# personalrobotics/or_cdchomp

Hardware: AMD Instinct MI355X
Metric: CHOMP iters/sec, 7-DOF x 100-waypoint (higher is better)
Workload: dtype f64; 1 GPU; WAM 7-DOF, n_points=100, batch=1024 random adofgoal per GPU, n_iter=100 per step, lambda=100 obs_factor=500, tabletop SDF 40x31x12 (BASELINE configs[1]); runs_per_gpu=1024, n_iter=100, n_points=100, dof=7, parallelism=runs sharded over 1 GPU(s) in contiguous blocks, no collective

## Files before the change

### or_cdchomp_amd/csrc/batch.cpp

```cpp
#include "module.h"
#include "kernel_table.h"
#include "launch.h"
#include "verdict_device.h"
#include <algorithm>
#include <cmath>
#include <cstring>
#include <functional>
#include <stdexcept>
#include <thread>
#include <exception>
#include <cstdlib>

hipError_t orc_launch_hmc_seed(uint32_t * state, int * next, const unsigned int * seeds, int n_runs, hipStream_t stream);
hipError_t orc_launch_hmc_plan_f64(uint32_t * state, int * next, int n_runs, int iter_begin, int iter_end, int cap, size_t mn, double lambda,
   double * noise, int * iters, int * overflow, hipStream_t stream);
hipError_t orc_launch_hmc_plan_f32(uint32_t * state, int * next, int n_runs, int iter_begin, int iter_end, int cap, size_t mn, double lambda,
   float * noise, int * iters, int * overflow, hipStream_t stream);
size_t orc_perturb_lds_bytes(int m, int n);
hipError_t orc_launch_perturb_f64(double * traj, int n_runs, int n_points, int n, int m, const unsigned int * seeds, int D,
   const double * genU, const double * genV, double scale, const double * lim_lo, const double * lim_hi, size_t lds, hipStream_t stream);
hipError_t orc_launch_perturb_f32(float * traj, int n_runs, int n_points, int n, int m, const unsigned int * seeds, int D,
   const double * genU, const double * genV, double scale, const double * lim_lo, const double * lim_hi, size_t lds, hipStream_t stream);
hipError_t orc_launch_select_best(const double * costs, const int * status, const unsigned long long * verdict_key, const int * group, int n_runs, int column,
   unsigned long long * key, int * count, int * best, hipStream_t stream);
// ... 479 lines not shown
   std::vector<int> flat((size_t) n_runs * maxr, -1);
   for (int k=0; k<n_runs; k++) for (size_t r=0; r<iters[k].size(); r++) flat[(size_t) k*maxr + r] = iters[k][r];
   if (flat.size() > hmc_cap_iters_)
   {
      own_hmc_iters_.reset(); own_hmc_iters_.reset(dev_alloc<int>(flat.size())); d_hmc_iters_ = own_hmc_iters_.as<int>(); hmc_cap_iters_ = flat.size();
   }
   hip_check(hipMemcpyAsync(d_hmc_iters_, flat.data(), flat.size()*sizeof(int), hipMemcpyHostToDevice, stream_), "hmc iters");
   const size_t ncount = (size_t) n_runs * maxr * mn;
   const size_t rsize = (params.precision == 64) ? 8 : 4;
   if (ncount * rsize > noise_cap_)
   {
      own_noise_.reset(); own_noise_.reset(dev_alloc<char>(ncount * rsize)); d_noise_ = own_noise_.as<void>(); noise_cap_ = ncount * rsize;
   }
   if (params.precision == 64)
   {
      std::vector<double> buf(ncount, 0.0);
      parallel_for_runs(n_runs, [&](int k_lo, int k_hi) {
         for (int k=k_lo; k<k_hi; k++) std::copy(noise[k].begin(), noise[k].end(), buf.begin() + (size_t) k*maxr*mn);
      });
      hip_check(hipMemcpyAsync(d_noise_, buf.data(), ncount*8, hipMemcpyHostToDevice, stream_), "noise");
      hip_check(hipStreamSynchronize(stream_), "noise sync");
   }
   else
   {
      std::vector<float> buf(ncount, 0.f);
      for (int k=0; k<n_runs; k++)
         for (size_t e=0; e<noise[k].size(); e++) buf[(size_t) k*maxr*mn + e] = (float) noise[k][e];
      hip_check(hipMemcpyAsync(d_noise_, buf.data(), ncount*4, hipMemcpyHostToDevice, stream_), "noise");
      hip_check(hipStreamSynchronize(stream_), "noise sync");
   }
}

template <typename real>
void BatchShard::launch(int n_iter, bool final_eval, bool carry)
{
   const IteratePlan & P = plan_;
   DevBatch<real> b;
   std::memset(&b, 0, sizeof(b));
   b.model = d_model_.as<const DevModel<real>>();
   b.sdfs = d_sdfs_.as<const DevSdf<real>>();
   b.sdfc = d_sdfc_.as<const DevSdfCell<real>>();
   b.n_sdfs = scn_.n_sdfs;
   b.scene_of_run = d_scene_of_run_.as<int>(); b.scene_nsdf = d_scene_nsdf_.as<int>(); b.n_scenes = scn_.n_scenes; b.sdfc_stride = scn_.sdfc_stride;
   b.n_runs = n_runs; b.n_points = m + 2; b.np_global = n_points; b.free_start = params.free_start; b.m = m; b.n = n;
   if (params.free_start && P.tile_first < 2)
      throw std::runtime_error("start_tsr: the first tile must hold the two points after the start point!");
   b.tile_m = P.tile_m;
   b.n_tiles = P.n_tiles; b.tile_first = P.tile_first; b.tile_rest = P.tile_rest;
   if (!P.g_in_lds && !d_Gcost_) d_Gcost_.reset(dev_alloc<real>((size_t) n_runs * m * n));
   b.traj = d_traj_.as<real>(); b.AG = d_AG_.as<real>(); b.Gcost = d_Gcost_.as<real>();
   b.Gdbg = sw_.debug_state ? d_G_.as<real>() : nullptr;
   b.g_in_lds = P.g_in_lds; b.lds_flags = P.lds_flags; b.t_in_lds = P.t_in_lds; b.t_staged = (P.lds_flags & ORC_LDS_T_STAGED) ? 1 : 0;
   b.ms = ms_;
   b.lay = P.lay;
   b.costs = d_costs_.as<double>(); b.trace = d_trace_.as<double>(); b.status = d_status_.as<int>(); b.iters_done = d_iters_done_.as<int>();
   b.leapfrog_first = d_leap_.as<int>();
   const double dt = 1.0/(n_points-1);
   b.dt = (real) dt;
   b.inv_2dt = (real)(1.0/(2.0*dt));
   b.inv_dt2 = (real)(1.0/(dt*dt));
   b.shared.lambda = (real) params.lambda;
   b.inv_m = (real)(1.0/m);
   b.shared.epsilon = (real) params.epsilon; b.epsilon_self = (real) params.epsilon_self;
   b.shared.obs_factor = (real) params.obs_factor; b.shared.obs_factor_self = (real) params.obs_factor_self;
   b.run_params = run_params_on_ ? d_run_params_.as<const RunParams<real>>() : nullptr;
   b.use_momentum = params.use_momentum; b.use_hmc = params.use_hmc && max_resamples_ > 0;
   b.D = (params.derivative == 1 && params.free_start) ? -1 : params.derivative;
   b.Aband = d_Aband_.as<const real>(); b.beta_s = d_beta_s_.as<const real>(); b.beta_g = d_beta_g_.as<const real>();
   b.metric64 = d_metric64_.as<const double>();
   b.kss = metric_.kss; b.ksg = metric_.ksg; b.kgg = metric_.kgg;
   b.solve_mode = met_.solve_mode;
   b.pcr_levels = metric_.pcr_levels;
   b.pcr = d_pcr_.as<const real>(); b.Ainv = d_Ainv_.as<const real>();
   b.ss_rank = (met_.solve_mode == 3) ? metric_.ss_rank : 0;
   b.jl_lo = d_jl_lo_.as<const real>(); b.jl_hi = d_jl_hi_.as<const real>();
   b.hmc_iters = d_hmc_iters_; b.noise = (const real *) d_noise_; b.max_resamples = max_resamples_;
   b.n_iter = n_iter; b.final_eval = final_eval ? 1 : 0; b.carry_status = carry ? 1 : 0;
   b.conv_patience = conv.patience > 0 ? conv.patience : 0;
   b.conv_rtol = conv.rtol; b.conv_obs_max = conv.obs_max;
   b.conv_prev = d_conv_prev_.as<double>(); b.conv_streak = d_conv_streak_.as<int>();
   b.phase_cycles = d_phase_.as<long long>();
   b.pcr_in_lds = P.pcr_in_lds; b.pcr_sym = met_.pcr_sym; b.pcr_rows = met_.pcr_rows; b.ag_in_lds = P.ag_in_lds;
   b.stagger_mode = sw_.stagger_mode; b.stagger_sleeps = sw_.stagger_sleeps; b.lim_generic = sw_.lim_generic;
   b.band_toeplitz = met_.band_toeplitz;
   for (int k=0; k<=ORC_SS_MAX_RANK; k++) { b.band_c64[k] = met_.band_c64[k]; b.band_c[k] = (real) met_.band_c64[k]; }
   if (params.derivative == 1 && m >= 2)
   {
      b.a_diag = (real) metric_.Adense[(size_t) 1*m + 1];
      b.a_off = (real) metric_.Adense[(size_t) 1*m + 0];
   }
   else if (params.derivative == 1)
   {
      b.a_diag = (real) metric_.Adense[0];
      b.a_off = (real) metric_.beta_s[0];
   }
   b.tsrs = d_tsrs_.as<const DevTsr<real>>(); b.n_tsrs = tsr_.n_tsrs; b.cons_k = tsr_.cons_k; b.tsr_blocks = tsr_.blocks;
   b.tsr_structured = P.tsr_structured; b.tsr_wcap = P.tsr_wcap; b.tsr_nmax = P.tsr_nmax;
   b.tsr_ws = d_tsr_ws_.as<real>(); b.tsr_ws_stride = tsr_.ws_stride; b.tsr_err = d_tsr_err_.as<int>();
   hipEvent_t ev[2] = { mod_->acquire_event(device), mod_->acquire_event(device) };
   hip_check(hipEventRecord(ev[0], stream_), "hipEventRecord");
   hipError_t e = orc_launch_iterate(b, P.lds_bytes, stream_, P.variant, P.block);
   hip_check(e, "chomp_iterate_kernel launch");
   hip_check(hipEventRecord(ev[1], stream_), "hipEventRecord");
   pending_events_.push_back(std::make_pair(ev[0], ev[1]));
}

void BatchShard::iterate_async(int n_iter, int iter_begin, bool final_eval, bool carry)
{
   if (n_iter < 0) throw std::runtime_error("n_iter must be >=0!");
   if (unusable_) throw std::runtime_error("hmc: an earlier iterate call of this batch ran out of room for its momentum resamples; destroy the batch and create it again!");
   DeviceGuard guard(device);
   last_n_iter = n_iter;
   const size_t tneed = (size_t) n_runs * (n_iter ? n_iter : 1) * 3;
   if (tneed > trace_cap_)
   {
      hip_check(hipStreamSynchronize(stream_), "sync");
      d_trace_.reset(); d_trace_.reset(dev_alloc<double>(tneed)); trace_cap_ = tneed;
   }
   max_resamples_ = 0;
   if (iter_begin == 0) std::fill(ext_noise_used_.begin(), ext_noise_used_.end(), 0);
   std::unique_lock<std::mutex> plan_lock;
   if (params.use_hmc && n_iter > 0 && hmc_on_device_) plan_lock = std::unique_lock<std::mutex>(mod_->plan_buffers(device, stream_).enqueue);
   if (params.use_hmc && n_iter > 0) plan_hmc(iter_begin, iter_begin + n_iter);
   if (params.precision == 64) launch<double>(n_iter, final_eval, carry); else launch<float>(n_iter, final_eval, carry);
}

void BatchShard::sync_begin(double * costs_out, int * status_out, int * iters_out)
{
   DeviceGuard guard(device);
   hipStream_t st = stream_;
   if (costs_out) hip_check(hipMemcpyAsync(costs_out, d_costs_.as<void>(), (size_t) n_runs*3*sizeof(double), hipMemcpyDeviceToHost, st), "costs");
   if (status_out) hip_check(hipMemcpyAsync(status_out, d_status_.as<void>(), n_runs*sizeof(int), hipMemcpyDeviceToHost, st), "status");
   if (iters_out) hip_check(hipMemcpyAsync(iters_out, d_iters_done_.as<void>(), n_runs*sizeof(int), hipMemcpyDeviceToHost, st), "iters_done");
   if (overflow_armed_)
   {
      hip_check(hipMemcpyAsync(&overflow_host_, d_overflow_.as<void>(), sizeof(int), hipMemcpyDeviceToHost, st), "hmc overflow");
      hip_check(hipMemsetAsync(d_overflow_.as<void>(), 0, sizeof(int), st), "hmc overflow");
   }
}

void BatchShard::sync_end()
{
   DeviceGuard guard(device);
   hip_check(hipStreamSynchronize(stream_), "hipStreamSynchronize");
   harvest_events(false);
   if (overflow_armed_ && overflow_host_)
   {
      overflow_host_ = 0;
      unusable_ = true;
      throw std::runtime_error("hmc: a run drew more momentum resamples in one iterate call than the plan has room for (probability ~1e-12 per run and call); "
                               "the batch is not usable any more: destroy it, create it again and iterate with fewer iterations per call!");
   }
}

namespace {
void download(void * d, size_t count, int precision, double * out, hipStream_t st)
{
   if (precision == 64)
   {
      hip_check(hipMemcpyAsync(out, d, count*sizeof(double), hipMemcpyDeviceToHost, st), "download");
      hip_check(hipStreamSynchronize(st), "sync");
   }
   else
   {
      std::vector<float> tmp(count);
      hip_check(hipMemcpyAsync(tmp.data(), d, count*sizeof(float), hipMemcpyDeviceToHost, st), "download");
// ... 519 lines not shown
```

### or_cdchomp_amd/csrc/chomp_kernel.hip

```cpp
#include <hip/hip_runtime.h>
#include <math.h>
#include <atomic>
#include <type_traits>
#include <utility>
#include "dev_types.h"
#include "kernel_table.h"
#include "launch.h"

#pragma clang fp contract(fast)


namespace {

#include "sdf_lookup.h"

__device__ __forceinline__ double rcp_fast(double x)
{
   double r = __builtin_amdgcn_rcp(x);
   r = fma(fma(-x, r, 1.0), r, r);
   r = fma(fma(-x, r, 1.0), r, r);
   return r;
}
__device__ __forceinline__ float rcp_fast(float x) { return 1.0f / x; }
__device__ __forceinline__ double sqrt_rsq(double x, double * inv)
// ... 1468 lines not shown
         __syncthreads();
      }
   }
   if (staged)
   {
      copy_batched<real, BLOCK>(E.traj_g + n, T_s + n, mn);
      __syncthreads();
   }
   phase_mark<real>(b, E, 4);
   if (b.phase_cycles && tid == 0) E.phc_s[6] += num_limadjs;
   return num_limadjs;
}

struct PassCosts { double obs, smooth; };
template <typename real, bool GS16, int BLOCK, int WGS = 0>
__device__ __attribute__((noinline)) PassCosts phase_costs(const void * kp, int do_iteration_in, double cost_lane)
{
   KArg<real> & b = *uniform_kernarg<real>(kp);
   const bool do_iteration = uni(do_iteration_in) != 0;
   const Env<real> E = make_env<real, GS16>(b, orc_smem);
   const int tid = threadIdx.x;
   const int n = b.n, m = b.m, np = b.n_points, mn = m*n;
   const float rn_f = 1.0f / (float) n;
   const real * T_s = E.T_u;
   const bool staged = !b.t_in_lds && b.t_staged;
   if (staged && !do_iteration)
   {
      copy_batched<real, BLOCK>(E.T_u, E.traj_g, np*n);
      __syncthreads();
   }
   PassCosts pc;
   __builtin_amdgcn_s_setprio(PRIO_UPDATE);
   {
      double acc = 0.0;
      if (b.D != 1) acc = band_cost_pass<real, BLOCK>(kp, E.pcr_tab, T_s);
      else
      for (int e=tid; e<mn; e+=BLOCK)
      {
         const int i = div_n(e, rn_f), c = e - i*n;
         const real sg = smooth_grad<real>(b, T_s, i, c);
         const real bt = b.a_off * ((i == 0 ? T_s[c] : (real)0) + (i == m-1 ? T_s[(np-1)*n + c] : (real)0));
         acc += (double) T_s[n + e] * (0.5 * ((double) sg + (double) bt));
      }
      double ss = 0.0, sg2 = 0.0, gg = 0.0;
      if (tid < n)
      {
         const double s0 = (double) T_s[tid], g0 = (double) T_s[(np-1)*n + tid];
         ss = s0*s0; sg2 = s0*g0; gg = g0*g0;
      }
      acc += 0.5 * (b.kss*ss + 2.0*b.ksg*sg2 + b.kgg*gg);
      const double a = wave_sum(cost_lane), c2 = wave_sum(acc);
      __syncthreads();
      if ((tid & 63) == 0) { E.red[tid >> 6] = a; E.red[8 + (tid >> 6)] = c2; }
      __syncthreads();
      pc.obs = sum_partials<BLOCK>(E.red);
      pc.smooth = sum_partials<BLOCK>(E.red + 8);
      pc.obs /= (double) m;
   }
   phase_mark<real>(b, E, 5);

   if (do_iteration && b.free_start)
   {
      real * Tw = E.T_s;
      if (tid < n) Tw[tid] = Tw[2*n + tid];
      __syncthreads();
   }
   if (do_iteration && E.mod.floating)
   {
      real * Tw = E.T_u;
      for (int w=tid; w<np; w+=BLOCK)
      {
         real * row = Tw + w*n;
         const real len = M<real>::sqrt_(row[3]*row[3] + row[4]*row[4] + row[5]*row[5] + row[6]*row[6]);
         const real inv = (real)1 / len;
         row[3] *= inv; row[4] *= inv; row[5] *= inv; row[6] *= inv;
         if (staged) { real * g = E.traj_g + w*n; g[3] = row[3]; g[4] = row[4]; g[5] = row[5]; g[6] = row[6]; }
      }
      __syncthreads();
   }
   if (b.conv_patience && do_iteration) conv_step<real>(b, pc.obs, pc.smooth);
   return pc;
}

template <typename real, bool GS16, int BLOCK, int WGS = 0>
__device__ __attribute__((noinline)) void phase_finish(const void * kp, int status_in, int iters_done_in, int leapfrog_first_in, int have_costs_in,
   double done_obs, double done_smooth)
{
   KArg<real> & b = *uniform_kernarg<real>(kp);
   int status = uni(status_in);
   const int iters_done = uni(iters_done_in), leapfrog_first = uni(leapfrog_first_in), have_costs = uni(have_costs_in);
   const Env<real> E = make_env<real, GS16>(b, orc_smem);
   const int run = blockIdx.x, tid = threadIdx.x;
   const int n = b.n, m = b.m, np = b.n_points, mn = m*n;
   __syncthreads();
   if (b.conv_patience)
   {
      const ConvState * cs = conv_state();
      if (status == 0 && uni(cs->streak) >= b.conv_patience) status = 1;
      if (tid == 0) { b.conv_prev[run] = cs->prev; b.conv_streak[run] = cs->streak; }
   }
   if (b.t_in_lds)
   {
      const int skip = b.free_start ? n : 0;
      for (int e=skip+tid; e<np*n; e+=BLOCK) E.traj_g[e - skip] = E.T_s[e];
   }
   if (b.use_momentum && b.ag_in_lds) for (int e=tid; e<mn; e+=BLOCK) E.AG_g[e] = E.AG_s[e];
   if (tid == 0)
   {
      if (b.phase_cycles) for (int k=0; k<8; k++) b.phase_cycles[(size_t) run*8 + k] = E.phc_s[k];
      if (have_costs)
      {
         b.costs[(size_t) run*3 + 0] = done_obs + done_smooth;
         b.costs[(size_t) run*3 + 1] = done_obs;
         b.costs[(size_t) run*3 + 2] = done_smooth;
      }
      b.status[run] = status;
      b.iters_done[run] = (b.carry_status ? b.iters_done[run] : 0) + iters_done;
      b.leapfrog_first[run] = leapfrog_first;
   }
   if (b.trace && status != 0)
      for (int e=iters_done*3 + tid; e<b.n_iter*3; e+=BLOCK)
         b.trace[(size_t) run * b.n_iter * 3 + e] = __longlong_as_double(0x7ff8000000000000LL);
}

template <typename real, bool TREE, bool GS16, int BLOCK, int KIND = 0, int WGS = 0>
__global__ __launch_bounds__(BLOCK, (WGS ? WGS : orc::waves_per_simd(sizeof(real), GS16, BLOCK)))
void chomp_iterate_kernel(const DevBatch<real> b)
{
   const void * kp = (const void *) __builtin_amdgcn_kernarg_segment_ptr();
   const int run = blockIdx.x;
   const int tid = threadIdx.x;

   if (b.carry_status && b.status[run] != 0 && (b.status[run] != 1 || b.n_iter != 0)) return;

   phase_setup<real, TREE, GS16, BLOCK, WGS>(kp);

   int leapfrog_first = uni(b.leapfrog_first[run]);
   int status = 0;
   int next_resample = 0;

   if (b.stagger_mode && b.stagger_mode != 9)
   {
      const bool late = (b.stagger_mode == 1) ? (blockIdx.x & 1) : ((blockIdx.x >> 8) & 1);
      if (late) for (int k=0; k<b.stagger_sleeps; k++) __builtin_amdgcn_s_sleep(127);
   }

   double done_obs = 0.0, done_smooth = 0.0;
   int have_costs = 0;
   int iters_done = 0;
   const int total_passes = b.n_iter + (b.final_eval ? 1 : 0);

   for (int it=0; it<total_passes; it++)
   {
      const bool do_iteration = (it < b.n_iter);
      if (do_iteration && uni(conv_state()->stop)) continue;

      if (do_iteration && b.use_hmc && b.use_momentum && next_resample < b.max_resamples
          && b.hmc_iters[(size_t) run * b.max_resamples + next_resample] == it)
      {
         phase_hmc<real, GS16, BLOCK, WGS>(kp, next_resample);
         leapfrog_first = 1;
         next_resample++;
      }

      double cost_lane = 0.0;
      for (int tk=0; tk<b.n_tiles; tk++)
      {
         const int ts = (tk == 0) ? 0 : b.tile_first + (tk - 1) * b.tile_rest;
         const int te = (tk == b.n_tiles - 1) ? b.m : b.tile_first + tk * b.tile_rest;
         if (b.stagger_mode == 9 && tk > 0) { if (tk == 1) for (int k=0; k<b.stagger_sleeps; k++) __builtin_amdgcn_s_sleep(10); continue; }
#ifndef ORC_ABLATE_FK
         if (!b.ms.fk_split && uni(tid >> 6) * 20 >= te - ts + 2) __syncthreads();
         else phase_fk<real, TREE, GS16, BLOCK, WGS>(kp, ts, te);
#ifdef ORC_ABLATE_FKTWICE
         phase_fk<real, TREE, GS16, BLOCK, WGS>(kp, ts, te);
#endif
#endif
#ifndef ORC_ABLATE_COST
         if (do_iteration && !GS16) cost_lane = phase_cost_body<real, TREE, GS16, BLOCK, KIND, true>(kp, ts, te, cost_lane);
         else
         cost_lane = do_iteration ? phase_cost<real, TREE, GS16, BLOCK, KIND, true, WGS>(kp, ts, te, cost_lane)
                                  : phase_cost<real, TREE, GS16, BLOCK, KIND, false, WGS>(kp, ts, te, cost_lane);
         if (tk == 0 && b.free_start) cost_lane = phase_cost_start<real, TREE, GS16, BLOCK, WGS>(kp, do_iteration ? 1 : 0, cost_lane);
#endif
      }

      if (do_iteration)
      {
         const bool lean = b.solve_mode == 2 && b.n <= 64 && !b.lim_generic && b.Gdbg == nullptr;
         const int num_limadjs = !lean ? uni(phase_update<real, TREE, GS16, BLOCK, WGS, 0>(kp, it, leapfrog_first))
                               : (b.n_tsrs == 0 ? uni(phase_update<real, TREE, GS16, BLOCK, WGS, 1>(kp, it, leapfrog_first))
                                                : uni(phase_update<real, TREE, GS16, BLOCK, WGS, 2>(kp, it, leapfrog_first)));
         if (b.use_momentum) leapfrog_first = 0;
         if (!(num_limadjs < 1000)) status = -1;
      }
      if (status != 0) break;

      PassCosts pc = phase_costs<real, GS16, BLOCK, WGS>(kp, do_iteration ? 1 : 0, cost_lane);
      pc.obs = unir(pc.obs); pc.smooth = unir(pc.smooth);

      if (tid == 0 && b.trace && do_iteration)
      {
         double * tr = b.trace + ((size_t) run * b.n_iter + it) * 3;
         tr[0] = pc.obs + pc.smooth; tr[1] = pc.obs; tr[2] = pc.smooth;
      }
      done_obs = pc.obs; done_smooth = pc.smooth; have_costs = 1;
      if (do_iteration) iters_done++;

   }

   phase_finish<real, GS16, BLOCK, WGS>(kp, status, iters_done, leapfrog_first, have_costs, done_obs, done_smooth);
}

template <typename real>
__global__ void seed_traj_kernel(real * traj, const double * starts, const double * goals,
   int n_runs, int n_points, int n, int floating)
{
   const long total = (long) n_runs * n_points;
   for (long idx = blockIdx.x * (long) blockDim.x + threadIdx.x; idx < total; idx += (long) gridDim.x * blockDim.x)
   {
      const int run = (int)(idx / n_points);
      const int i = (int)(idx - (long) run * n_points);
      double row[ORC_MAX_JOINTS + 7];
      for (int j=0; j<n; j++)
      {
         const double s = starts[(size_t) run*n + j];
         const double g = goals[(size_t) run*n + j];
         row[j] = s + (g - s) * i / (n_points - 1);
      }
      if (floating)
      {
         const double len = ::sqrt(__dadd_rn(__dadd_rn(__dadd_rn(__dmul_rn(row[3], row[3]), __dmul_rn(row[4], row[4])), __dmul_rn(row[5], row[5])), __dmul_rn(row[6], row[6])));
         const double inv = 1.0 / len;
         row[3] *= inv; row[4] *= inv; row[5] *= inv; row[6] *= inv;
      }
      for (int j=0; j<n; j++) traj[((size_t) run * n_points + i) * n + j] = (real) row[j];
   }
}

template <typename real, bool TREE>
__global__ __launch_bounds__(ORC_BLOCK)
void collision_verdict_kernel(DevVerdict<real> v)
{
   extern __shared__ __align__(16) unsigned char smem_raw[];
   const DevModel<real> & gmod = *v.model;
   const int run = blockIdx.x, tid = threadIdx.x;
   const int n = v.n, np = v.n_points, nj = gmod.nj, Sa = gmod.Sa;
   const int pstr = (Sa*3) | 1, astr = (nj*6) | 1, chunk = v.chunk;
   const int scene = v.scene_of_run ? v.scene_of_run[run] : 0;
   const int n_fields = v.scene_nsdf ? v.scene_nsdf[scene] : v.n_sdfs;
   const DevSdf<real> * sdfs = v.sdfs + (size_t) scene * v.n_sdfs;
   unsigned long long * key_s = (unsigned long long *) smem_raw;
   real * lds = (real *)(smem_raw + 16);
   real * rows_s = lds;
   real * pos_s = rows_s + ((chunk*n + 3) & ~3);
   real * ax_s = pos_s + ((chunk*pstr + 3) & ~3);
   real * base_s = ax_s + ((chunk*astr + 3) & ~3);
   real * srad_s = base_s + 12;
   int * slot_s = (int *)(srad_s + ((Sa + 3) & ~3));
   int * xml_s = slot_s + ((gmod.Sa_real + 3) & ~3);
   int * jctl_s = xml_s + ((Sa + 3) & ~3);
   for (int e=tid; e<12; e+=ORC_BLOCK) base_s[e] = (e < 9) ? gmod.base_R[e] : gmod.base_t[e-9];
   for (int e=tid; e<Sa; e+=ORC_BLOCK) { srad_s[e] = gmod.sph_radius[e]; xml_s[e] = v.slot_xml[e]; }
   for (int e=tid; e<gmod.Sa_real; e+=ORC_BLOCK) slot_s[e] = gmod.slot_of[e];
   for (int e=tid; e<nj; e+=ORC_BLOCK) { jctl_s[2*e] = gmod.joints[e].packed; jctl_s[2*e+1] = 0; }
   if (tid == 0) key_s[0] = ORC_VERDICT_NONE;
   ModelView<real> mod;
   mod.nj = nj; mod.n = n; mod.floating = gmod.floating; mod.tree = gmod.tree; mod.Sa = Sa; mod.S = gmod.S; mod.GS = gmod.GS;
   mod.base_sph_begin = gmod.base_sph_begin; mod.base_sph_end = gmod.base_sph_end; mod.jt_scan = 0;
   mod.Sa_real = gmod.Sa_real; mod.placed = gmod.placed; mod.live_mask = gmod.live_mask; mod.slot_of = slot_s;
   mod.base_R = base_s; mod.base_t = base_s + 9;
   mod.jctl = jctl_s; mod.sph_affects = nullptr; mod.n_static = 0; mod.empty_mask = 0u;
   mod.jpk = (const __attribute__((address_space(4))) int *) gmod.jpacked;
   mod.jpk2 = (const __attribute__((address_space(4))) int *) gmod.jpacked2;
   mod.sph_pos_c = (const __attribute__((address_space(4))) real (*)[3]) gmod.sph_pos;
   mod.joints_c = (const __attribute__((address_space(4))) DevJoint<real> *) gmod.joints;
   mod.slot_c = (const __attribute__((address_space(4))) int *) gmod.slot_of;
   mod.fkj = (const __attribute__((address_space(4))) DevFkJoint<real> *) gmod.fkj;
   __syncthreads();

   const real * traj = v.traj + (size_t) run * np * n;
   const int s0 = v.offs[run], s1 = v.offs[run+1];
   double my_depth = 0.0; unsigned long long my_key = ORC_VERDICT_NONE;
   for (int base=s0; base<s1; base+=chunk)
   {
      const int count = (s1 - base < chunk) ? s1 - base : chunk;
      for (int e=tid; e<count*n; e+=ORC_BLOCK)
      {
         const int s = e / n, c = e - s*n;
         const int sg = v.seg[base + s];
         const real uu = v.u[base + s];
// ... 145 lines not shown
```

### or_cdchomp_amd/csrc/dev_types.h

```cpp
#pragma once
#include <cstddef>

#define ORC_MAX_JOINTS   32
#define ORC_MAX_SPHERES  64
#define ORC_MAX_POINTS   4096
#define ORC_MAX_SAVE     4
#define ORC_MAX_SDFS     8
#define ORC_BLOCK        256
#ifndef ORC_WGS_PER_CU
#define ORC_WGS_PER_CU    3
#endif
#ifndef ORC_WGS_PER_CU_FP32_MANY
#define ORC_WGS_PER_CU_FP32_MANY 4
#endif
#define ORC_SS_MAX_RANK   4
#define ORC_SCAN_RPL      4
#define ORC_VERDICT_NONE  0x7fffffffffffffffull
#define ORC_LDS_HEADER    256
#define ORC_LIM_LIST      64
#define ORC_LIM_SCRATCH  (256 + ORC_LIM_LIST*16)
#define ORC_PAIR_ROUNDS   16
#define ORC_PAIR_DEG      4

enum : int
// ... 150 lines not shown
struct RunParams
{
   real lambda, epsilon, obs_factor, obs_factor_self;
};

template <typename real>
struct DevBatch
{
   ModelScalars ms;
   LdsLayout lay;
   const DevModel<real> * model;
   const DevSdf<real> * sdfs;
   const DevSdfCell<real> * sdfc;
   int n_sdfs;
   const int * scene_of_run;
   const int * scene_nsdf;
   int n_scenes, sdfc_stride;
   int n_runs, n_points, m, n;
   int tile_m;
   int n_tiles;
   int tile_first, tile_rest;
   real * traj;
   real * AG;
   real * Gdbg;
   real * Gcost;
   double * costs;
   double * trace;
   int * status;
   int * iters_done;
   int * leapfrog_first;
   real dt, inv_2dt, inv_dt2, inv_m;
   real epsilon_self;
   RunParams<real> shared;
   const RunParams<real> * run_params;
   int use_momentum, use_hmc, D;
   const real * Aband;
   const real * beta_s;
   const real * beta_g;
   const double * metric64;
   double kss, ksg, kgg;
   int solve_mode;
   int pcr_levels;
   const real * pcr;
   const real * Ainv;
   const real * jl_lo;
   const real * jl_hi;
   const int * hmc_iters;
   const real * noise;
   int max_resamples;
   int n_iter;
   int final_eval;
   int carry_status;
   long long * phase_cycles;
   real a_diag, a_off;
   int pcr_in_lds;
   int t_in_lds;
   int t_staged;
   int g_in_lds;
   int lds_flags;
   int ag_in_lds;
   int pcr_sym;
   int pcr_rows;
   int lim_generic;
   int stagger_mode;
   int stagger_sleeps;
   const DevTsr<real> * tsrs;
   int n_tsrs, cons_k;
   int tsr_blocks;
   int tsr_structured;
   int tsr_wcap;
   int tsr_nmax;
   int free_start, np_global;
   real * tsr_ws;
   size_t tsr_ws_stride;
   int * tsr_err;
   int band_toeplitz;
   real band_c[ORC_SS_MAX_RANK + 1];
   double band_c64[ORC_SS_MAX_RANK + 1];
   int ss_rank;
   int conv_patience;
   double conv_rtol, conv_obs_max;
   double * conv_prev;
   int * conv_streak;
};

template <typename real>
struct DevVerdict
{
   const DevModel<real> * model;
   const DevSdf<real> * sdfs;
   int n_sdfs;
   const int * scene_of_run;
   const int * scene_nsdf;
   int n_runs, n_points, n;
   int chunk;
   const real * traj;
   const int * offs;
   const int * seg;
   const real * u;
   const int * slot_xml;
   int n_pairs;
   const int * pairs;
   const real * pair_rsum;
   const real * inact_pos;
   unsigned long long * key_out;
   double * depth_out;
};


template <typename real>
struct ModelView
{
   int nj, n, floating, tree, Sa, S, GS, base_sph_begin, base_sph_end, jt_scan, Sa_real, placed, n_static;
   unsigned int empty_mask;
   unsigned long long live_mask;
   const int * slot_of;
   const real * base_R;
   const real * base_t;
   const int * jctl;
   const unsigned long long * sph_affects;
   const unsigned long long * sph_allowed;
   const __attribute__((address_space(4))) int * jpk;
   const __attribute__((address_space(4))) int * jpk2;
   const __attribute__((address_space(4))) real (* sph_pos_c)[3];
   const __attribute__((address_space(4))) int * slot_c;
   const __attribute__((address_space(4))) DevJoint<real> * joints_c;
   const __attribute__((address_space(4))) DevFkJoint<real> * fkj;
   const __attribute__((address_space(4))) int * static_slot_c;
   const __attribute__((address_space(4))) real (* static_pos_c)[3];
   const __attribute__((address_space(4))) RunParams<real> * rp;
   int n_sdfs;
   const __attribute__((address_space(4))) DevSdfCell<real> * sdfc;
};
#if defined(__HIPCC__)
__host__ __device__
#endif
#define ORC_LDS_SMALL_WORK 1
#define ORC_LDS_G_GLOBAL   2
#define ORC_LDS_T_GLOBAL   4
#define ORC_LDS_T_STAGED   8
inline LdsLayout lds_layout(int np, int n, int Sa, int S, int nj, int tile_m, int pcr_rows, int real_size,
   int use_ag, int n_sdfs, int sdf_size, int flags, int pair_entries = 0)
{
   const int m = np - 2, mn = m*n;
   LdsLayout L;
   int o = 0;
   auto take = [&o](int count) { const int at = o; o += (count + 3) & ~3; return at; };
   L.pstr = (Sa*3) | 1;
   L.astr = (nj*6) | 1;
   const int lim_reals = ((ORC_LIM_SCRATCH + real_size - 1) / real_size + 3) & ~3;
   const int work_min = 1280/real_size;
   const int work_reals = ((((flags & ORC_LDS_SMALL_WORK) || mn <= work_min) ? work_min : mn) + 3) & ~3;
   const int tile_reals = (((tile_m+2)*L.pstr + 3) & ~3) + (((tile_m+2)*L.astr + 3) & ~3);
   const bool g_global = (flags & ORC_LDS_G_GLOBAL) != 0;
   const bool t_staged = (flags & ORC_LDS_T_GLOBAL) && (flags & ORC_LDS_T_STAGED);
   const bool alias = tile_reals >= work_reals + lim_reals + (g_global ? ((mn + 3) & ~3) : 0) + (t_staged ? ((np*n + 3) & ~3) : 0);
   L.T = (flags & ORC_LDS_T_GLOBAL) ? 0 : take(np*n);
   L.G = g_global ? 0 : take(mn);
   L.W = alias ? 0 : take(work_reals);
   L.AG = take(use_ag ? mn : 0);
   L.pos = take((tile_m+2)*L.pstr);
   L.ax = take((tile_m+2)*L.astr);
   if (alias) L.W = L.pos;
   if (g_global) L.G = L.pos + work_reals + lim_reals;
   L.Tu = t_staged ? L.pos + work_reals + lim_reals + (g_global ? ((mn + 3) & ~3) : 0) : -1;
   L.srad = take(S);
// ... 21 lines not shown
```

### or_cdchomp_amd/csrc/fold.cpp

```cpp
#include "stages.h"
#include "kernel_table.h"
#include <algorithm>
#include <cmath>
#include <cstdio>
#include <cstdlib>
#include <cstring>
#include <functional>
#include <stdexcept>

namespace orc {

Switches Switches::read()
{
   Switches s;
   auto on = [](const char * name) { return getenv(name) != nullptr; };
   auto num = [](const char * name) { Int v; if (const char * e = getenv(name)) { v.set = true; v.value = atoi(e); } return v; };
   auto num_or = [&num](const char * name, int otherwise) { const Int v = num(name); return v.set ? v.value : otherwise; };
   s.debug_plan = on("ORC_DEBUG_PLAN"); s.phase_timers = on("ORC_PHASE_TIMERS"); s.debug_state = on("ORC_DEBUG_STATE");
   s.hmc_device = on("ORC_HMC_DEVICE"); s.hmc_host = on("ORC_HMC_HOST"); s.hmc_plan_sync = on("ORC_HMC_PLAN_SYNC");
   s.no_jt_scan = on("ORC_NO_JT_SCAN"); s.no_placement = on("ORC_NO_PLACEMENT"); s.no_static_lanes = on("ORC_NO_STATIC_LANES");
   s.pairs_chain64_only = on("ORC_PAIRS_CHAIN64_ONLY"); s.no_pairs = on("ORC_NO_PAIRS"); s.no_kind = on("ORC_NO_KIND");
   s.no_fk_split = on("ORC_NO_FK_SPLIT"); s.no_semisep = on("ORC_NO_SEMISEP"); s.no_scan_solve = on("ORC_NO_SCAN_SOLVE");
   s.pcr_full = on("ORC_PCR_FULL"); s.no_short128 = on("ORC_NO_SHORT128"); s.no_band_toeplitz = on("ORC_NO_BAND_TOEPLITZ");
   s.tsr_dense = on("ORC_TSR_DENSE");
   const Int staged = num("ORC_T_STAGED");
   s.t_staged_off = staged.set && staged.value == 0;
   s.lim_generic = num_or("ORC_LIM_GENERIC", 0); s.stagger_mode = num_or("ORC_STAGGER_MODE", 0); s.stagger_sleeps = num_or("ORC_STAGGER_SLEEPS", 10);
   s.scan_max_m = num_or("ORC_SCAN_MAX_M", 1 << 30); s.wgs128 = num_or("ORC_WGS128", 8);
   s.block_threads = num("ORC_BLOCK_THREADS"); s.tile_m = num("ORC_TILE_M"); s.pcr_lds = num("ORC_PCR_LDS"); s.ag_lds = num("ORC_AG_LDS");
   s.wgs = num("ORC_WGS"); s.g_lds = num("ORC_G_LDS"); s.t_lds = num("ORC_T_LDS"); s.hmc_room = num("ORC_HMC_ROOM");
   return s;
}

int JointTree::attach_of(const Robot & robot, int link) const
{
   for (int li=link; li>=0; li=robot.parent[li]) if (link2joint[li] >= 0) return link2joint[li];
   return -1;
}

JointTree fold_joint_tree(const Robot & robot, bool floating_base)
{
   JointTree T;
   const int n_adof = (int) robot.active_dofs.size();
   const int col0 = floating_base ? 7 : 0;
   T.link2joint.assign(robot.n_links, -1);
   for (int li=0; li<robot.n_links; li++)
   {
      if (robot.joint_type[li] == 0) continue;
      for (int j=0; j<n_adof; j++)
         if (robot.active_dofs[j] == robot.dof_index[li])
         {
            for (int lk : T.jlink)
               if (robot.dof_index[lk] == robot.dof_index[li])
                  throw std::runtime_error("two joints share one active dof (mimic joints are not supported)!");
            T.link2joint[li] = (int) T.jlink.size();
            T.jlink.push_back(li); T.jcol.push_back(col0 + j);
         }
   }
   const int nj = T.nj();
   if (nj > ORC_MAX_JOINTS) throw std::runtime_error("too many active joints for this build!");
   T.jparent.resize(nj);
   for (int k=0; k<nj; k++)
   {
      const int pl = robot.parent[T.jlink[k]];
      T.jparent[k] = (pl >= 0) ? T.attach_of(robot, pl) : -1;
   }
   T.children.resize(nj);
   for (int k=0; k<nj; k++) { if (T.jparent[k] < 0) T.roots.push_back(k); else T.children[T.jparent[k]].push_back(k); }
   T.load_slot.assign(nj, -1); T.save_slot.assign(nj, -1);
   std::vector<int> need(nj, 0);
   std::function<int(int)> slots_needed = [&](int k) -> int
   {
      std::vector<int> & ch = T.children[k];
      for (int c : ch) slots_needed(c);
      std::stable_sort(ch.begin(), ch.end(), [&](int a, int b) { return need[a] < need[b]; });
      int v = 0;
      for (size_t c=0; c<ch.size(); c++) v = std::max(v, need[ch[c]] + ((c + 1 < ch.size()) ? 1 : 0));
      return need[k] = v;
   };
   for (int rk : T.roots) slots_needed(rk);
   int open_slots = 0;
   std::function<void(int)> visit = [&](int k)
   {
      T.order.push_back(k);
      const size_t nc = T.children[k].size();
      if (nc > 1)
      {
         if (open_slots >= ORC_MAX_SAVE) throw std::runtime_error("kinematic tree branches too deeply for this build!");
         T.save_slot[k] = open_slots++;
      }
      for (size_t c=0; c<nc; c++)
      {
         if (nc > 1 && c + 1 == nc) open_slots--;
         T.load_slot[T.children[k][c]] = (c == 0) ? -1 : T.save_slot[k];
         visit(T.children[k][c]);
      }
   };
   for (int rk : T.roots) { T.load_slot[rk] = -2; visit(rk); }
   T.pos_in_order.resize(nj);
   for (int k=0; k<nj; k++) T.pos_in_order[T.order[k]] = k;
   return T;
}

Xform local_moved(const Robot & robot, int li)
{
   Xform x = xform_from_pose(robot.pose_parent_joint[li]);
   if (robot.joint_type[li] == 1)
// ... 727 lines not shown
```

### or_cdchomp_amd/csrc/plan.cpp

```cpp
#include "stages.h"
#include "kernel_table.h"
#include <algorithm>
#include <cmath>
#include <cstdio>
#include <stdexcept>

namespace orc {

namespace {

const size_t LDS_PER_CU = 160*1024;
const size_t LDS_GRANULE = 1280;
const double FK_WAYPOINTS_PER_WAVE = 20.0;
const double FK_PASS_PER_JOINT = 1.7e3;
const double ROUND_GS16 = 11e3;
const double ROUND_PAIRS = 9e3;
const double ROUND_PER_SPHERE = 350.0;
const double FIXED_PER_ITERATION = 30e3;
const double PCR_THROUGH_L2 = 1e3, AG_GLOBAL = 2e3, G_GLOBAL = 2e3, T_GLOBAL_STAGED = 4e3, T_GLOBAL_IN_PLACE = 12e3;
const double PER_EXTRA_WAVE = 0.05;
const double SHAPE_192 = 0.90;

struct Shape { int block, wgs; };

// ... 75 lines not shown
{
   P.n_tiles = (m + P.tile_m - 1) / P.tile_m;
   P.tile_first = P.tile_rest = P.tile_m;
   const int unit = std::max(1, P.block / lanes_per_wp);
   const int full = (P.tile_m / unit) * unit;
   if (full > 0 && P.n_tiles > 1)
   {
      const int first = m - full * (P.n_tiles - 1);
      auto rounds = [&](int a, int rest) {
         int r = (a + unit - 1) / unit, left = m - a;
         for (int k=1; k<P.n_tiles; k++) { const int v = std::min(rest, left); r += (v + unit - 1) / unit; left -= v; }
         return r;
      };
      if (first > 0 && first <= P.tile_m && rounds(first, full) < rounds(P.tile_m, P.tile_m)) { P.tile_first = first; P.tile_rest = full; }
   }
}

void size_tsr_solve(IteratePlan & P, const PlanInput & in, const Switches & sw)
{
   if (in.n_tsrs == 0 || in.derivative != 1 || sw.tsr_dense) return;
   const int N = in.n + in.tsr_kmax, Wd = N + in.n + 1;
   const size_t need = (size_t) N * Wd + (size_t) in.n * (in.n + 1) + in.n + (size_t)(in.tsr_kmax + 2) * sizeof(int) / in.real_bytes + 2;
   const size_t have = (size_t)(P.tile_m + 2) * P.lay.astr;
   if (Wd <= 64 && need <= have) { P.tsr_structured = 1; P.tsr_wcap = N * Wd; P.tsr_nmax = N; }
}

}

IteratePlan plan_iterate(const PlanInput & in, const Switches & sw)
{
   const int variant = in.variant;
   auto has = [&](int var, int block) { return kernel_exists(kernel_of(var, block, (int) in.real_bytes)); };
   const int max_wgs_budget = waves_per_simd((int) in.real_bytes, in.GS == 16, 256);
   const int max_wgs_default = sw.wgs.set ? sw.wgs.value : max_wgs_budget;
   int force_block_asked = in.module_threads ? in.module_threads : in.params_threads;
   if (force_block_asked == 512 && !has(variant, 512)) force_block_asked = 0;
   int want_wgs = in.module_per_cu ? in.module_per_cu : in.params_per_cu;
   const bool can128 = has(variant, 128);
   if (want_wgs == 0 && ((in.n_tsrs > 0 && !(variant & ORC_VAR_FLOATING)) || (variant & ORC_VAR_PAIRS) || (in.overlapping && !(variant & ORC_VAR_FLOATING)))) want_wgs = 4;
   if (want_wgs == 3) want_wgs = 0;
   const bool short128 = in.m <= 32 && !sw.no_short128;
   const bool planner128 = force_block_asked == 0 && ((in.overlapping && in.n_tsrs > 0) || short128) && can128 && !in.free_start && !sw.block_threads.set;
   const bool kernels_at_4 = has(variant | ORC_VAR_WGS4, 256);

   IteratePlan P;
   bool budget4 = false;
   for (int pass=(planner128 ? -1 : 0); pass<3 && !P.tile_m; pass++)
   {
      const bool relax = (pass == 2);
      int max_wgs = relax ? max_wgs_budget : max_wgs_default;
      Forced force;
      force.block = (pass == -1) ? 128 : force_block_asked;
      if (!relax) { force.tile = sw.tile_m.set ? sw.tile_m.value : 0; force.pcr = sw.pcr_lds.set ? sw.pcr_lds.value : -1; force.ag = sw.ag_lds.set ? sw.ag_lds.value : -1; }
      budget4 = (pass == 0) && (want_wgs == 4) && kernels_at_4 && (force.block == 0 || force.block == 256)
                && !sw.block_threads.set && !sw.wgs.set && !sw.tile_m.set;
      if (budget4) { max_wgs = 4; force.block = 256; }
      if (sw.block_threads.set && !relax) force.block = sw.block_threads.value;
      if (sw.g_lds.set && !relax) force.g = sw.g_lds.value;
      if (sw.t_lds.set && !relax) force.tl = sw.t_lds.value;
      P = IteratePlan();
      double best_score = -1.0;
      const std::vector<Shape> shapes = shapes_of(in, sw, max_wgs, budget4, force.block, can128);
      if (force.block == 128 && !can128) force.block = 0;
      for (const Shape & sh : shapes)
      {
         if (force.block && sh.block != force.block) continue;
         for (int with_pcr=1; with_pcr>=0; with_pcr--)
            for (int ag_lds=1; ag_lds>=0; ag_lds--)
               for (int g_lds=1; g_lds>=0; g_lds--)
                  for (int t_lds=1; t_lds>=0; t_lds--)
                  {
                     const Option o = { with_pcr, ag_lds, g_lds, t_lds };
                     if (option_allowed(in, force, o)) try_option(in, sw, force, sh, o, P, best_score);
                  }
      }
   }
   if (!P.tile_m) throw std::runtime_error("run does not fit the LDS of one CU!");
   P.variant = variant | (budget4 ? ORC_VAR_WGS4 : 0);
   cut_tiles(P, in.m, (in.GS == 16) ? 16 : in.GS);
   P.lay = lds_layout(in.m + 2, in.n, in.Sa, in.S, in.nj, P.tile_m, P.pcr_in_lds ? in.pcr_rows : 0, (int) in.real_bytes,
                      in.use_momentum && P.ag_in_lds, in.n_sdfs, (int) in.sdf_bytes, P.lds_flags, in.pair_entries);
   size_tsr_solve(P, in, sw);
   if (sw.debug_plan)
      fprintf(stderr, "orc plan: %d threads per workgroup, tile_m %d (%d tiles, first of %d) lds %zu bytes (%d workgroups per CU) pcr_in_lds %d ag_in_lds %d g_in_lds %d t_in_lds %d solve_mode %d\n", P.block, P.tile_m,
              P.n_tiles, P.tile_first, P.lds_bytes, P.workgroups_per_cu(), P.pcr_in_lds, P.ag_in_lds, P.g_in_lds, P.t_in_lds, in.solve_mode);
   return P;
}

}
```

### or_cdchomp_amd/csrc/stages.h

```cpp
#pragma once
#include <map>
#include <memory>
#include <mutex>
#include <string>
#include <vector>
#include "dev_types.h"
#include "host_math.h"

namespace orc {

struct Robot
{
   std::string name;
   int n_links = 0;
   std::vector<int> parent;
   std::vector<Pose> pose_parent_joint;
   std::vector<int> joint_type;
   std::vector<double> axis;
   std::vector<int> dof_index;
   int n_dof = 0;
   std::vector<double> limit_lower, limit_upper;
   std::vector<double> limit_vel;
   struct Sphere { int link; double pos[3]; double radius; int body = 0; };
   std::vector<Sphere> spheres;
   std::vector<std::string> link_names;
   struct Manip { std::string name; int link; Pose tool; };
   std::vector<Manip> manips;
   int active_manip = 0;
   std::vector<std::pair<int, int>> adjacent;
   bool self_check = true;
   struct Grab { std::string body; int link; Xform rel; std::vector<unsigned char> touch_link; std::vector<std::string> touch_body; };
   std::vector<Grab> grabbed;
   Pose transform;
   std::vector<double> dof_values;
   std::vector<int> active_dofs;
   bool does_affect(int dof, int link) const;
   std::vector<unsigned char> self_pairs_excluded() const;
   std::vector<unsigned char> run_self_pairs_excluded(int n_own) const;
   void fk(const Pose & base, const std::vector<double> & q, std::vector<Xform> & frames) const;
};

struct Sdf
{
   std::string kinbody_name;
   Pose pose;
   Grid grid;
   std::map<int, std::shared_ptr<void>> dev64, dev32;
};

struct ScenePlacement
{
   std::shared_ptr<Sdf> sdf;
   Pose pose_world_kinbody;
};
struct SceneTable
{
   std::vector<std::vector<ScenePlacement>> scenes;
   std::vector<int> scene_of_run;
   int max_fields() const;
};

struct TsrSpec
{
   int ee_link = -1;
   Pose tool;
   Pose T0w, Twe;
   double Bw[6][2];
   int point = -1;
};

struct BatchParams
{
   std::vector<TsrSpec> tsrs;
   int free_start = 0;
   int n_points = 101;
   int floating_base = 0;
   double lambda = 10.0;
   int derivative = 1;
   int use_momentum = 0;
   int use_hmc = 0;
   double hmc_resample_lambda = 0.02;
   double epsilon = 0.1, epsilon_self = 0.04, obs_factor = 200.0, obs_factor_self = 10.0;
   int precision = 64;
   int workgroup_threads = 0;
   int workgroups_per_cu = 0;
};

struct Switches
{
   struct Int { bool set = false; int value = 0; };
   bool debug_plan = false, phase_timers = false, debug_state = false, hmc_device = false, hmc_host = false, hmc_plan_sync = false;
   bool no_jt_scan = false, no_placement = false, no_static_lanes = false, pairs_chain64_only = false, no_pairs = false;
   bool no_kind = false, no_fk_split = false, no_semisep = false, no_scan_solve = false, pcr_full = false, no_short128 = false;
   bool no_band_toeplitz = false, tsr_dense = false;
   bool t_staged_off = false;
   int lim_generic = 0, stagger_mode = 0, stagger_sleeps = 10, scan_max_m = 1 << 30, wgs128 = 8;
   Int block_threads, tile_m, pcr_lds, ag_lds, wgs, g_lds, t_lds, hmc_room;
   static Switches read();
};

struct JointTree
{
   std::vector<int> jlink, jcol;
   std::vector<int> link2joint;
   std::vector<int> jparent;
   std::vector<std::vector<int>> children;
   std::vector<int> roots;
   std::vector<int> order, pos_in_order;
   std::vector<int> load_slot, save_slot;
   int nj() const { return (int) jlink.size(); }
   int attach_of(const Robot & robot, int link) const;
};
JointTree fold_joint_tree(const Robot & robot, bool floating_base);
Xform local_moved(const Robot & robot, int li);
Xform fixed_between(const Robot & robot, int from_link, int li);
void point_in(const Robot & robot, int from_link, int li, const double * pin, double * pout);

struct PlacementCache { std::map<std::string, std::vector<int>> & placed; std::recursive_mutex & mutex; };
std::string placement_key(const Robot & robot, const BatchParams & params, int n_static);

template <typename real>
struct FoldedModel
{
   std::unique_ptr<DevModel<real>> model;
   ModelScalars scalars;
   std::vector<int> device_sphere_order;
   std::vector<int> slot_xml;
   int pair_entries = 0;
   int variant = 0;
};
template <typename real>
FoldedModel<real> fold_robot(const Robot & robot, const BatchParams & params, int n, const JointTree & tree, int asked_block,
   const Switches & sw, PlacementCache cache);

struct TsrDims
{
   int n_tsrs = 0;
   int cons_k = 0;
   int blocks = 0;
   int kmax = 0;
   size_t ws_stride = 0;
};
template <typename real>
struct FoldedTsrs : TsrDims { std::vector<DevTsr<real>> tsrs; };
template <typename real>
FoldedTsrs<real> fold_tsrs(const Robot & robot, const BatchParams & params, const JointTree & tree, int m, int n);

struct SceneDims { int n_scenes = 1, n_sdfs = 0, sdfc_stride = 0; };
template <typename real>
struct FoldedScenes : SceneDims
{
   std::vector<DevSdf<real>> sdfs;
   std::vector<DevSdfCell<real>> cells;
   std::vector<int> scene_nsdf;
   bool one_aligned = false;
   struct GridSlot { int scene, field; Sdf * sdf; };
   std::vector<GridSlot> grids;
};
template <typename real>
FoldedScenes<real> fold_scenes(const SceneTable & table, int run0, int n_runs, bool offsets_24bit);

struct MetricDims
{
   int solve_mode = 0;
   int pcr_rows = 0, pcr_sym = 0;
   int band_toeplitz = 0;
   double band_c64[ORC_SS_MAX_RANK + 1] = { 0.0 };
};
struct MetricTables : MetricDims
{
   std::vector<double> pcr;
   bool pcr_as_doubles = false;
   std::vector<double> metric64;
   std::vector<double> Ainv;
};
MetricTables pack_metric(const Metric & metric, const BatchParams & params, int m, size_t real_bytes, const Switches & sw);

struct PlanInput
// ... 25 lines not shown
```

Before: 18.27 million CHOMP iterations/s.

## Compute previous iteration's cost on an idle wavefront during forward kinematics

The per-iteration cost reduction pass (phase_costs) is removed from the critical path. The previous iteration's smoothness cost and obstacle-cost reduction are now computed by the last wavefront, which sits idle while the other wavefronts run forward kinematics. Wave partial sums are stashed in LDS and handed over through spare LDS words, and trace writes are deferred by one iteration. A final explicit cost pass covers the last iteration. This removes a barrier-heavy stage per iteration in exchange for complex gating conditions and extra global reads of the trajectory.

```diff
diff --git a/or_cdchomp_amd/csrc/batch.cpp b/or_cdchomp_amd/csrc/batch.cpp
--- a/or_cdchomp_amd/csrc/batch.cpp
+++ b/or_cdchomp_amd/csrc/batch.cpp
@@ -585,6 +585,7 @@
    b.phase_cycles = d_phase_.as<long long>();
    b.pcr_in_lds = P.pcr_in_lds; b.pcr_sym = met_.pcr_sym; b.pcr_rows = met_.pcr_rows; b.ag_in_lds = P.ag_in_lds;
    b.stagger_mode = sw_.stagger_mode; b.stagger_sleeps = sw_.stagger_sleeps; b.lim_generic = sw_.lim_generic;
+   b.no_idle_costs = sw_.no_idle_costs ? 1 : 0;
    b.band_toeplitz = met_.band_toeplitz;
    for (int k=0; k<=ORC_SS_MAX_RANK; k++) { b.band_c64[k] = met_.band_c64[k]; b.band_c[k] = (real) met_.band_c64[k]; }
    if (params.derivative == 1 && m >= 2)
diff --git a/or_cdchomp_amd/csrc/chomp_kernel.hip b/or_cdchomp_amd/csrc/chomp_kernel.hip
--- a/or_cdchomp_amd/csrc/chomp_kernel.hip
+++ b/or_cdchomp_amd/csrc/chomp_kernel.hip
@@ -1574,6 +1574,48 @@
    return pc;
 }
 
+constexpr int IDLE_COSTS_BATCH = 4;
+template <typename real, int BLOCK, int WGS = 0>
+__device__ __attribute__((noinline)) void phase_costs_lone(const void * kp)
+{
+   KArg<real> & b = *uniform_kernarg<real>(kp);
+   const int lane = threadIdx.x & 63;
+   const int n = b.n, m = b.m, np = b.n_points, mn = m*n;
+   const real * T = b.traj + (size_t) blockIdx.x * np * n;
+   double * red = (double *) orc_smem;
+   __builtin_amdgcn_s_setprio(PRIO_COST);
+   double acc = 0.0;
+   for (int k0=0; k0<mn; k0+=IDLE_COSTS_BATCH*64)
+   {
+      real tl[IDLE_COSTS_BATCH], tc[IDLE_COSTS_BATCH], tr[IDLE_COSTS_BATCH];
+#pragma unroll
+      for (int q=0; q<IDLE_COSTS_BATCH; q++)
+      {
+         const int e = k0 + q*64 + lane, ec = (e < mn) ? e : 0;
+         tl[q] = T[ec]; tc[q] = T[ec + n]; tr[q] = T[ec + 2*n];
+      }
+#pragma unroll
+      for (int q=0; q<IDLE_COSTS_BATCH; q++)
+      {
+         const int e = k0 + q*64 + lane;
+         const real sg = b.a_diag * tc[q] + b.a_off * (tl[q] + tr[q]);
+         const real bt = b.a_off * ((e < n ? tl[q] : (real)0) + (e >= mn - n ? tr[q] : (real)0));
+         const double term = (double) tc[q] * (0.5 * ((double) sg + (double) bt));
+         acc += (e < mn) ? term : 0.0;
+      }
+   }
+   double ss = 0.0, sg2 = 0.0, gg = 0.0;
+   if (lane < n)
+   {
+      const double s0 = (double) T[lane], g0 = (double) T[(np-1)*n + lane];
+      ss = s0*s0; sg2 = s0*g0; gg = g0*g0;
+   }
+   acc += 0.5 * (b.kss*ss + 2.0*b.ksg*sg2 + b.kgg*gg);
+   const double smooth = wave_sum(acc);
+   const double obs = sum_partials<BLOCK>(red) / (double) m;
+   if (lane == 0) { red[8] = obs; red[9] = smooth; }
+}
+
 template <typename real, bool GS16, int BLOCK, int WGS = 0>
 __device__ __attribute__((noinline)) void phase_finish(const void * kp, int status_in, int iters_done_in, int leapfrog_first_in, int have_costs_in,
    double done_obs, double done_smooth)
@@ -1641,6 +1683,23 @@
    int have_costs = 0;
    int iters_done = 0;
    const int total_passes = b.n_iter + (b.final_eval ? 1 : 0);
+#ifdef ORC_ABLATE_FK
+   constexpr bool IDLE_COSTS = false;
+#else
+   constexpr bool IDLE_COSTS = GS16 && !TREE;
+#endif
+   static_assert(BLOCK <= 512, "red[wave] holds the wavefronts' partial sums next to the hand-over words red[8], red[9]");
+   const bool idle_costs = IDLE_COSTS && !b.no_idle_costs && !b.t_in_lds && b.t_staged && b.n_tsrs == 0 && !b.ms.fk_split && !b.ms.floating && !b.free_start
+      && b.conv_patience == 0 && !b.use_hmc && b.D == 1 && b.solve_mode == 2 && b.n <= 64 && !b.lim_generic && b.Gdbg == nullptr && b.stagger_mode != 9
+      && (BLOCK/64 - 1) * 20 >= (b.n_tiles == 1 ? b.m : b.tile_first) + 2;
+   auto take_costs = [&](int row, double obs, double smooth) {
+      if (tid == 0 && b.trace && row >= 0)
+      {
+         double * tr = b.trace + ((size_t) run * b.n_iter + row) * 3;
+         tr[0] = obs + smooth; tr[1] = obs; tr[2] = smooth;
+      }
+      done_obs = obs; done_smooth = smooth; have_costs = 1;
+   };
 
    for (int it=0; it<total_passes; it++)
    {
@@ -1662,12 +1721,22 @@
          const int te = (tk == b.n_tiles - 1) ? b.m : b.tile_first + tk * b.tile_rest;
          if (b.stagger_mode == 9 && tk > 0) { if (tk == 1) for (int k=0; k<b.stagger_sleeps; k++) __builtin_amdgcn_s_sleep(10); continue; }
 #ifndef ORC_ABLATE_FK
-         if (!b.ms.fk_split && uni(tid >> 6) * 20 >= te - ts + 2) __syncthreads();
+         if (!b.ms.fk_split && uni(tid >> 6) * 20 >= te - ts + 2)
+         {
+            if constexpr (IDLE_COSTS) if (idle_costs && tk == 0 && it > 0 && uni(tid >> 6) == BLOCK/64 - 1) phase_costs_lone<real, BLOCK, WGS>(kp);
+            __syncthreads();
+         }
          else phase_fk<real, TREE, GS16, BLOCK, WGS>(kp, ts, te);
 #ifdef ORC_ABLATE_FKTWICE
          phase_fk<real, TREE, GS16, BLOCK, WGS>(kp, ts, te);
 #endif
 #endif
+         if constexpr (IDLE_COSTS) if (idle_costs && tk == 0 && it > 0 && tid == 0 && b.trace)
+         {
+            const double * red = (const double *) orc_smem;
+            double * tr = b.trace + ((size_t) run * b.n_iter + (it - 1)) * 3;
+            tr[0] = red[8] + red[9]; tr[1] = red[8]; tr[2] = red[9];
+         }
 #ifndef ORC_ABLATE_COST
          if (do_iteration && !GS16) cost_lane = phase_cost_body<real, TREE, GS16, BLOCK, KIND, true>(kp, ts, te, cost_lane);
          else
@@ -1677,6 +1746,11 @@
 #endif
       }
 
+      if constexpr (IDLE_COSTS) if (idle_costs && do_iteration)
+      {
+         const double a = wave_sum(cost_lane);
+         if ((tid & 63) == 0) ((double *) orc_smem)[tid >> 6] = a;
+      }
       if (do_iteration)
       {
          const bool lean = b.solve_mode == 2 && b.n <= 64 && !b.lim_generic && b.Gdbg == nullptr;
@@ -1688,17 +1762,21 @@
       }
       if (status != 0) break;
 
-      PassCosts pc = phase_costs<real, GS16, BLOCK, WGS>(kp, do_iteration ? 1 : 0, cost_lane);
-      pc.obs = unir(pc.obs); pc.smooth = unir(pc.smooth);
-
-      if (tid == 0 && b.trace && do_iteration)
-      {
-         double * tr = b.trace + ((size_t) run * b.n_iter + it) * 3;
-         tr[0] = pc.obs + pc.smooth; tr[1] = pc.obs; tr[2] = pc.smooth;
-      }
-      done_obs = pc.obs; done_smooth = pc.smooth; have_costs = 1;
+      if (!(idle_costs && do_iteration))
+      {
+         PassCosts pc = phase_costs<real, GS16, BLOCK, WGS>(kp, do_iteration ? 1 : 0, cost_lane);
+         take_costs(do_iteration ? it : -1, unir(pc.obs), unir(pc.smooth));
+      }
       if (do_iteration) iters_done++;
 
+   }
+   if constexpr (IDLE_COSTS) if (idle_costs && status != 0 && iters_done > 0)
+      take_costs(-1, unir(((const double *) orc_smem)[8]), unir(((const double *) orc_smem)[9]));
+   if constexpr (IDLE_COSTS) if (idle_costs && status == 0 && !b.final_eval && b.n_iter > 0)
+   {
+      const double cl = ((tid & 63) == 0) ? ((const double *) orc_smem)[tid >> 6] : 0.0;
+      PassCosts pc = phase_costs<real, GS16, BLOCK, WGS>(kp, 1, cl);
+      take_costs(b.n_iter - 1, unir(pc.obs), unir(pc.smooth));
    }
 
    phase_finish<real, GS16, BLOCK, WGS>(kp, status, iters_done, leapfrog_first, have_costs, done_obs, done_smooth);
diff --git a/or_cdchomp_amd/csrc/dev_types.h b/or_cdchomp_amd/csrc/dev_types.h
--- a/or_cdchomp_amd/csrc/dev_types.h
+++ b/or_cdchomp_amd/csrc/dev_types.h
@@ -256,6 +256,7 @@
    double conv_rtol, conv_obs_max;
    double * conv_prev;
    int * conv_streak;
+   int no_idle_costs;
 };
 
 template <typename real>
diff --git a/or_cdchomp_amd/csrc/fold.cpp b/or_cdchomp_amd/csrc/fold.cpp
--- a/or_cdchomp_amd/csrc/fold.cpp
+++ b/or_cdchomp_amd/csrc/fold.cpp
@@ -22,7 +22,7 @@
    s.pairs_chain64_only = on("ORC_PAIRS_CHAIN64_ONLY"); s.no_pairs = on("ORC_NO_PAIRS"); s.no_kind = on("ORC_NO_KIND");
    s.no_fk_split = on("ORC_NO_FK_SPLIT"); s.no_semisep = on("ORC_NO_SEMISEP"); s.no_scan_solve = on("ORC_NO_SCAN_SOLVE");
    s.pcr_full = on("ORC_PCR_FULL"); s.no_short128 = on("ORC_NO_SHORT128"); s.no_band_toeplitz = on("ORC_NO_BAND_TOEPLITZ");
-   s.tsr_dense = on("ORC_TSR_DENSE");
+   s.tsr_dense = on("ORC_TSR_DENSE"); s.no_idle_costs = on("ORC_NO_IDLE_COSTS");
    const Int staged = num("ORC_T_STAGED");
    s.t_staged_off = staged.set && staged.value == 0;
    s.lim_generic = num_or("ORC_LIM_GENERIC", 0); s.stagger_mode = num_or("ORC_STAGGER_MODE", 0); s.stagger_sleeps = num_or("ORC_STAGGER_SLEEPS", 10);
diff --git a/or_cdchomp_amd/csrc/plan.cpp b/or_cdchomp_amd/csrc/plan.cpp
--- a/or_cdchomp_amd/csrc/plan.cpp
+++ b/or_cdchomp_amd/csrc/plan.cpp
@@ -181,8 +181,9 @@
                       in.use_momentum && P.ag_in_lds, in.n_sdfs, (int) in.sdf_bytes, P.lds_flags, in.pair_entries);
    size_tsr_solve(P, in, sw);
    if (sw.debug_plan)
-      fprintf(stderr, "orc plan: %d threads per workgroup, tile_m %d (%d tiles, first of %d) lds %zu bytes (%d workgroups per CU) pcr_in_lds %d ag_in_lds %d g_in_lds %d t_in_lds %d solve_mode %d\n", P.block, P.tile_m,
-              P.n_tiles, P.tile_first, P.lds_bytes, P.workgroups_per_cu(), P.pcr_in_lds, P.ag_in_lds, P.g_in_lds, P.t_in_lds, in.solve_mode);
+      fprintf(stderr, "orc plan: %d threads per workgroup, tile_m %d (%d tiles, first of %d) lds %zu bytes (%d workgroups per CU) pcr_in_lds %d ag_in_lds %d g_in_lds %d t_in_lds %d solve_mode %d t_staged %d\n", P.block, P.tile_m,
+              P.n_tiles, P.tile_first, P.lds_bytes, P.workgroups_per_cu(), P.pcr_in_lds, P.ag_in_lds, P.g_in_lds, P.t_in_lds, in.solve_mode,
+              (P.lds_flags & ORC_LDS_T_STAGED) ? 1 : 0);
    return P;
 }
 
diff --git a/or_cdchomp_amd/csrc/stages.h b/or_cdchomp_amd/csrc/stages.h
--- a/or_cdchomp_amd/csrc/stages.h
+++ b/or_cdchomp_amd/csrc/stages.h
@@ -94,6 +94,7 @@
    bool no_kind = false, no_fk_split = false, no_semisep = false, no_scan_solve = false, pcr_full = false, no_short128 = false;
    bool no_band_toeplitz = false, tsr_dense = false;
    bool t_staged_off = false;
+   bool no_idle_costs = false;
    int lim_generic = 0, stagger_mode = 0, stagger_sleeps = 10, scan_max_m = 1 << 30, wgs128 = 8;
    Int block_threads, tile_m, pcr_lds, ag_lds, wgs, g_lds, t_lds, hmc_room;
    static Switches read();
```

After: 18.67 million CHOMP iterations/s (median of 6 runs). 2.2% higher.
